# cityflow-project/CityFlow

Hardware: AMD Instinct MI355X
Metric: vehicle_steps_per_sec (higher is better)
Workload: dtype f64; 1 GPU; grid_30x30 (reference generator, --tlPlan, interval 1.0) + 3000 seeded interior flows (1 veh / 6 s each until t=240 s); single engine; running_vehicles_start=96748, running_vehicles_end=71131, lanes=11160, lane_count_hash_end=cf8592fdc74305bd, backend=hip-gfx950, layout=ring, parallelism=1 gpu

## Files before the change

### cityflow_amd/csrc/hip/cfx_device.h

```cpp
#pragma once

#include <hip/hip_runtime.h>
#include <stdint.h>

#include "cityflow_amd.h"

#define CFX_INT_MAX 2147483647

struct DevNet {
    int R, L, K, I, E;
    const double *drvLength, *drvMaxSpeed, *xDist, *phaseTime;
    const int32_t *laneRoad, *laneIndex, *laneLLStart, *laneLL, *llStartLane, *llEndLane, *llInter, *llRoadLink, *llType,
        *llXStart, *xPeer, *xLL, *interVirtual, *interNRL, *interPhaseStart, *interAvailStart;
    const uint8_t *phaseAvail;
    const int32_t *xPeerBit;
    const int32_t *llLocal;
    const int32_t *interMaskStart;
    const double2 *drvLM;
    const double2 *xDD;
    const int4 *xPack;
    const int4 *llPack;
    const int4 *laneLL4;
    const int4 *laneEnd4;
    const uint8_t *laneGhost;
// ... 107 lines not shown
        for (int k = 0; k < 8; ++k) curSpeedSum += v[k];
    }
    {
        double v[8];
#pragma unroll
        for (int k = 0; k < 8; ++k) v[k] = i + k < n ? speedAt(i + k) : 0.0;
#pragma unroll
        for (int k = 0; k < 8; ++k)
            if (i + k < n) curSpeedSum += v[k];
    }
    speedSum += curSpeedSum;
    int tail = head + len;
    if (tail >= kLaneHistoryMax) tail -= kLaneHistoryMax;
    h.num[(size_t) tail * h.L + lane] = n;
    h.avg[(size_t) tail * h.L + lane] = n ? curSpeedSum / n : 0;
    h.head[lane] = head;
    h.len[lane] = len + 1;
    h.hNum[lane] = hn;
    h.hAvg[lane] = hn ? speedSum / hn : 0;
}

struct TailRec {
    double dis, speed;
    int32_t slot, templ, prevDrv, tag;
};
static_assert(sizeof(TailRec) == 32, "tail record layout");

struct LLAux {
    double uDis, uSpeed, fDis, fSpeed, llLen, startLen;
    int32_t uTempl, fTempl;
};
static_assert(sizeof(LLAux) == 56, "laneLink aux record layout");

struct LeaverPrefetch {
    bool valid;
    double nextLen;
    int vid, route, routePos;
    bool prevValid;
    int prevDrv;
    int templP1;
    int blockerVidP2;
};

constexpr int kFlagCustom = 1, kFlagLastRoad = 2, kFlagStateGap = 4;
#ifndef CFX_CROSS2_WAVES
#define CFX_CROSS2_WAVES 7
#endif
struct StepCtx {
    static constexpr int kCross2Waves = CFX_CROSS2_WAVES;
    DevNet n;
    DevTables t;
    SlotArrays s;
    const int32_t *segStart;
    const int32_t *cnt;
    const int32_t *admitStep;
    int admissionsVisible;
    const int32_t *curPhase;
    const int32_t *oldToNew;
    const int32_t *vPriority;
    const double *vCustomSpeed;
    const double *vGapState;
    int4 *llDyn;
    unsigned long long *interMask;
    int2 *llGate;
    int32_t *laneTail;
    int2 *admitRec;
// ... 251 lines not shown
```

### cityflow_amd/csrc/hip/cfx_hip.hip

```cpp
#include <hip/hip_runtime.h>
#include <hip/hip_ext.h>

#include <algorithm>
#include <atomic>
#include <chrono>
#include <cmath>
#include <cstdio>
#include <cstring>
#include <map>
#include <string>
#include <thread>
#include <type_traits>
#include <vector>


#include "cfx_kernels.h"
#include "cfx_lc_kernels.h"
#include "cfx_ring_kernels.h"
#include "cfx_dense_kernels.h"

#ifndef CFX_CROSS2_BLOCKS_PER_CU
#define CFX_CROSS2_BLOCKS_PER_CU 7
#endif

// ... 174 lines not shown
        const int road = hLaneRoad[lane], base = hRouteStart[route], len = hRouteStart[route + 1] - base;
        int p = 0;
        while (p < len && hRouteRoads[base + p] != road) ++p;
        int next = -1;
        if (p < len) {
            const int ll = hNextLL[hNextStart[base + p] + hLaneIndex[lane]];
            next = ll < 0 ? -1 : L + ll;
        }
        if (next >= 0) return next;
        return (len > 0 && hRouteRoads[base + len - 1] == road) ? -2 : -1;
    }
    std::vector<int2> hRingGeo;
    size_t ringSlots = 0;
    double ringMinLen = 0.0;
    int ringScale = 1;
    int ringG = 14, ringCalm = 0, ringHold = 0;
    int2 *dRingGeo = nullptr;
    int32_t *rHead = nullptr, *rCnt = nullptr, *slotOf = nullptr;
    int4 *rScratch = nullptr;
    SlotArrays rs{};
    double2 *rKin[2] = {nullptr, nullptr};
    int4 *rMeta = nullptr;
    int rcur = 0;
    int2 *rBlk[2] = {nullptr, nullptr};
    TailRec *rTail[2] = {nullptr, nullptr}, *rTailNow = nullptr;
    MoverRec *rMovers = nullptr;
    long long *rFinKey = nullptr;
    int32_t *rFinVid = nullptr;
    double *rFinTerm = nullptr;
    int rFinCap = 0, rJobCap = 0;
    int32_t *rJobs = nullptr;
    RingJob *rJobRecs = nullptr;
    LLAux *rLLAux = nullptr;
    int4 *rLLGate = nullptr;
    int32_t *rGatePhase = nullptr;
    int4 *rList = nullptr;
    size_t rListCap = 0;
    int32_t *rListCount = nullptr;
    unsigned long long *rIdxGranules = nullptr;
    RingDense rd{};
    size_t rdCap = 0;
    int32_t *rOff = nullptr;

    bool timesDyadic = true;
    static bool dyadic(double x) { return x * 1024.0 == std::nearbyint(x * 1024.0) && std::fabs(x) < 4398046511104.0; }
    bool exactTimes() const {
        if (!timesDyadic) return false;
        const double cum = mirrorValid ? hMirror->sc.cumulativeTravelTime : cumLoaded;
        return dyadic(cum) && cum < 1099511627776.0;
    }
    double cumLoaded = 0.0;

    int64_t step = 0;
    int64_t finishedKnown = 0;
    int64_t finishedOffset = 0;

    bool profiling = false;
    std::vector<hipEvent_t> evPool;
    std::vector<int> evKernel;
    size_t evUsed = 0;
    double profMs[kNumProfKernels] = {};
    int64_t profLaunches[kNumProfKernels] = {};
    const char *slotSymbol[kNumProfKernels] = {};
    cfx_host_stats hostStats{};
    int stallCause = 0;

// ... 263 lines not shown
        RingCtx c{};
        c.tailR = rTail[(step + 1) & 1];
        c.tailW = rTail[step & 1];
        c.tailNow = rTailNow;
        c.betweenSteps = stepping ? 0 : 1;
        c.n = net;
        c.t.templ = dTempl.p;
        c.t.nTempl = (int) hTempl.size();
        c.t.routeStart = dRouteStart.p;
        c.t.routeRoads = dRouteRoads.p;
        c.t.nextStart = dNextStart.p;
        c.t.nextLL = dNextLL.p;
        c.s = rs;
        c.kin = rKin[rcur];
        c.kinN = rKin[rcur ^ 1];
        c.meta = rMeta;
        c.blkR = rBlk[(step + 1) & 1];
        c.blkW = rBlk[step & 1];
        c.slotOf = slotOf;
        c.vState = vt.state;
        c.ringGeo = dRingGeo;
        c.head = rHead;
        c.cnt = rCnt;
        c.admitStep = admitStep;
        c.curPhase = curPhase;
        c.vPriority = vt.priority;
        c.vCustomSpeed = vt.customSpeed;
        c.vGapState = vt.gapState;
        c.llDyn = llDyn;
        c.interMask = interMask;
        c.llGate = rLLGate;
        c.gatePhase = rGatePhase;
        c.llAux = rLLAux;
        c.laneTail = laneTail;
        c.admitRec = admitRec;
        c.step = (int32_t) step;
        c.interval = cfg.interval;
        return c;
    }
    template <typename T> int freeRaw(T **p) {
        if (*p) {
            forget(*p);
            HIP_TRY(hipFree(*p));
            *p = nullptr;
        }
        return CFX_OK;
    }
    int ringFree() {
        int rc = 0;
        rc |= freeRaw(&rs.vid) | freeRaw(&rs.drv) | freeRaw(&rs.prevDrv) | freeRaw(&rs.routePos) | freeRaw(&rs.route) |
              freeRaw(&rBlk[0]) | freeRaw(&rBlk[1]) | freeRaw(&rKin[0]) | freeRaw(&rKin[1]) | freeRaw(&rMeta) | freeRaw(&rMovers) |
              freeRaw(&dRingGeo) | freeRaw(&rJobs) | freeRaw(&rJobRecs);
        return rc ? CFX_ERR_DEVICE : CFX_OK;
    }
    int ringAllocate(double minLen) {
        hRingGeo.resize((size_t) D);
        size_t run = 0;
        for (int d = 0; d < D; ++d) {
            double want = std::ceil(hDrvLength[d] / minLen) + 6.0;
            if (cfg.ring_capacity_percent > 0) want = std::max(2.0, want * cfg.ring_capacity_percent / 100.0);
            want *= ringScale;
            size_t cap = 8;
            while ((double) cap < want && cap < (1u << (kRingIdxBits - 1))) cap <<= 1;
            run = (run + cap - 1) & ~(cap - 1);
            hRingGeo[d] = make_int2((int) run, (int) cap - 1);
            run += cap;
            if (run > 0x7fff0000u) return fail("ring layout: more than 2^31 slots");
        }
        ringSlots = run;
        ringMinLen = minLen;
        int rc;
#define RALLOC(ptr) if ((rc = allocRaw(&ptr, ringSlots))) return rc;
        RALLOC(rs.vid) RALLOC(rs.drv) RALLOC(rs.prevDrv) RALLOC(rs.routePos) RALLOC(rs.route)
        RALLOC(rBlk[0]) RALLOC(rBlk[1]) RALLOC(rKin[0]) RALLOC(rKin[1]) RALLOC(rMeta) RALLOC(rMovers)
#undef RALLOC
        HIP_TRY(hipMemsetAsync(rBlk[0], 0xFF, ringSlots * sizeof(int2), stream));
        HIP_TRY(hipMemsetAsync(rBlk[1], 0xFF, ringSlots * sizeof(int2), stream));
        HIP_TRY(hipMemsetAsync(rMeta, 0, ringSlots * sizeof(int4), stream));
        if ((rc = upload(&dRingGeo, hRingGeo.data(), hRingGeo.size()))) return rc;
        rJobCap = (int) std::max<size_t>(4096, ringSlots / 8);
        if ((rc = allocRaw(&rJobs, (size_t) rJobCap * kJobShards))) return rc;
        if ((rc = allocRaw(&rJobRecs, (size_t) rJobCap * kJobShards))) return rc;
        if (!rHead) {
            if ((rc = allocRaw(&rHead, (size_t) D + 1))) return rc;
            if ((rc = allocRaw(&rCnt, (size_t) D + 1))) return rc;
            if ((rc = allocRaw(&rOff, (size_t) D + 2))) return rc;
            if ((rc = allocRaw(&rScratch, (size_t) D))) return rc;
            if ((rc = allocRaw(&rTail[0], (size_t) D))) return rc;
            if ((rc = allocRaw(&rTail[1], (size_t) D))) return rc;
            if ((rc = allocRaw(&rTailNow, (size_t) D))) return rc;
            if ((rc = allocRaw(&rLLAux, (size_t) K))) return rc;
            if ((rc = allocRaw(&rLLGate, (size_t) K))) return rc;
            if ((rc = allocRaw(&rGatePhase, (size_t) 2 * std::max(I, 1)))) return rc;
            HIP_TRY(hipMemsetAsync(rGatePhase, 0xFF, (size_t) 2 * std::max(I, 1) * sizeof(int32_t), stream));
            rFinCap = std::max(1 << 16, L * 8);
            if ((rc = allocRaw(&rFinKey, (size_t) rFinCap))) return rc;
            if ((rc = allocRaw(&rFinVid, (size_t) rFinCap))) return rc;
            if ((rc = allocRaw(&rFinTerm, (size_t) rFinCap))) return rc;
            HIP_TRY(hipMemsetAsync(rCnt, 0, ((size_t) D + 1) * sizeof(int32_t), stream));
        }
        return CFX_OK;
    }
    int ensureDense(size_t n) {
        if (n <= rdCap) return CFX_OK;
        const size_t nc = std::max<size_t>(n + n / 4, 1 << 14);
        int rc;
        HIP_TRY(hipStreamSynchronize(stream));
#define DGROW(ptr) if ((rc = freeRaw(&ptr)) || (rc = allocRaw(&ptr, nc))) return rc;
        DGROW(rd.vid) DGROW(rd.drv) DGROW(rd.prevDrv) DGROW(rd.blockerVid) DGROW(rd.enterLLT) DGROW(rd.routePos) DGROW(rd.leaderVid)
        DGROW(rd.flags) DGROW(rd.dis) DGROW(rd.speed) DGROW(rd.gap)
#undef DGROW
        rdCap = nc;
        return CFX_OK;
    }
    int ringGather(bool wantLeader, int32_t *totalOut) {
        hipLaunchKernelGGL(kr_offsets, dim3(1), dim3(kOffBlock), 0, stream, (const int32_t *) rCnt, rOff, D + 1);
        int32_t total = 0;
        HIP_TRY(hipMemcpyAsync(&total, rOff + D, sizeof(int32_t), hipMemcpyDeviceToHost, stream));
        HIP_TRY(hipStreamSynchronize(stream));
        int rc = ensureDense((size_t) total);
        if (rc) return rc;
        if (total) hipLaunchKernelGGL(kr_gather, dim3(gridFor(D)), dim3(kBlock), 0, stream, rctx(), (const int32_t *) rOff, rd, wantLeader ? 1 : 0);
        HIP_TRY(hipGetLastError());
        *totalOut = total;
        return CFX_OK;
    }
    int ringClearStepTags() {
        HIP_TRY(hipMemsetAsync(rTailNow, 0xFF, (size_t) D * sizeof(TailRec), stream));
        HIP_TRY(hipMemsetAsync(interMask, 0, (size_t) std::max(nMaskWords, 1) * sizeof(unsigned long long), stream));
        return CFX_OK;
    }
    bool ringMerge = true;
    bool commitPending = false;
    size_t activeEstimate() const {
        const unsigned long long pr = __atomic_load_n(&hMirror->progress, __ATOMIC_RELAXED);
        return (size_t) (pr & 0xFFFFFFFFu) + (size_t) nQueueLanes * 4;
    }
    RingCommit commitArgs(size_t activeEst, bool lightsDone, int *nStatOut) {
        const int nStat = (int) std::min<size_t>(std::max<size_t>(1, activeEst >> 16), 64);
        *nStatOut = nStat;
        return RingCommit{rScratch, rMovers, waitHead, curPhase, remain, (int) cfg.rl_traffic_light, (int) nMaskWords,
                          sc, rFinKey, rFinVid, rFinTerm, rFinCap, jobCount,
                          hMirror, finTicket, nStat, vt.state, slotOf, exactTimes() ? 1 : 0,
                          lightsDone ? 1 : 0, publishTo(), finCount};
    }
    bool haloImportPending = false;
    RingHaloIn pendingImport{};
    bool histPending = false;
    RingHist takeHist(int firstBlock) {
        RingHist rh{};
        rh.firstBlock = 0x7fffffff;
        if (hist.num && ring && histPending) {
            rh.h = hist;
            rh.firstBlock = firstBlock;
            histPending = false;
        }
        return rh;
    }
    int settle(bool withHistory = true) {
        if (haloImportPending) {
            haloImportPending = false;
// ... 2542 lines not shown
    e->devObserveIdle = 0;
    return CFX_OK;
}

int32_t cfx_get_intersection_features(cfx_engine *e, int32_t *phase, double *remain, int32_t *in, int32_t *inWaiting, int32_t *out,
                                      int32_t *inside, int32_t *pressure, int32_t maxRoadLinks, int32_t maxPhases) {
    if (!e || (!phase && !remain && !in && !inWaiting && !out && !inside && !pressure)) return CFX_ERR_INVALID;
    auto fail = [e](const std::string &m) { return e->fail(m); };
    HIP_TRY(hipSetDevice(e->device));
    int rc;
    if ((rc = interPrepare(e, maxRoadLinks, maxPhases, "cfx_get_intersection_features"))) return rc;
    const size_t nI = (size_t) e->I, nM = nI * e->interTab.M, nP = nI * e->interTab.P;
    if (!e->interOutI && (rc = e->allocRaw(&e->interOutI, nI + 4 * nM + nP))) return rc;
    if (!e->interOutD && (rc = e->allocRaw(&e->interOutD, nI))) return rc;
    int32_t *dPhase = e->interOutI, *dIn = dPhase + nI, *dWait = dIn + nM, *dOut = dWait + nM, *dInside = dOut + nM,
            *dPressure = dInside + nM;
    launchInterFeatures(e, phase ? dPhase : nullptr, remain ? e->interOutD : nullptr, in ? dIn : nullptr, inWaiting ? dWait : nullptr,
                        out ? dOut : nullptr, inside ? dInside : nullptr, pressure ? dPressure : nullptr);
    HIP_TRY(hipGetLastError());
    auto back = [&](void *dst, const void *src, size_t bytes) {
        return (dst && bytes) ? hipMemcpyAsync(dst, src, bytes, hipMemcpyDeviceToHost, e->stream) : hipSuccess;
    };
    HIP_TRY(back(phase, dPhase, nI * sizeof(int32_t)));
    HIP_TRY(back(remain, e->interOutD, nI * sizeof(double)));
    HIP_TRY(back(in, dIn, nM * sizeof(int32_t)));
    HIP_TRY(back(inWaiting, dWait, nM * sizeof(int32_t)));
    HIP_TRY(back(out, dOut, nM * sizeof(int32_t)));
    HIP_TRY(back(inside, dInside, nM * sizeof(int32_t)));
    HIP_TRY(back(pressure, dPressure, nP * sizeof(int32_t)));
    HIP_TRY(hipStreamSynchronize(e->stream));
    return CFX_OK;
}

int32_t cfx_profile_kernel_count(void) { return kNumProfKernels; }
const char *cfx_profile_kernel_name(int32_t k) { return (k >= 0 && k < kNumProfKernels) ? kProfNames[k] : ""; }

int32_t cfx_profile_enable(cfx_engine *e, int32_t on) {
    if (!e) return CFX_ERR_INVALID;
    (void) hipSetDevice(e->device);
    if (e->profiling && !on) e->profCollect();
    e->profiling = on != 0;
    return CFX_OK;
}

int32_t cfx_profile_read(cfx_engine *e, double *totalMs, int64_t *launches) {
    if (!e) return CFX_ERR_INVALID;
    (void) hipSetDevice(e->device);
    e->profCollect();
    for (int k = 0; k < kNumProfKernels; ++k) {
        if (totalMs) totalMs[k] = e->profMs[k];
        if (launches) launches[k] = e->profLaunches[k];
        e->profMs[k] = 0;
        e->profLaunches[k] = 0;
    }
    return CFX_OK;
}

}
```

### cityflow_amd/csrc/hip/cfx_ring_kernels.h

```cpp
#pragma once

#include <type_traits>

#include "cfx_kernels.h"


namespace cfxd {

struct RingCtx {
#ifndef CFX_RING_CROSS2_WAVES
#define CFX_RING_CROSS2_WAVES 5
#endif
    static constexpr int kCross2Waves = CFX_RING_CROSS2_WAVES;
    DevNet n;
    DevTables t;
    SlotArrays s;
    double2 *kin;
    double2 *kinN;
    int4 *meta;
    const int2 *blkR;
    int2 *blkW;
    int32_t *slotOf;
    const uint8_t *vState;
    const int2 *ringGeo;
    const TailRec *tailR;
    TailRec *tailW;
    TailRec *tailNow;
    int betweenSteps;
    int32_t *head;
    int32_t *cnt;
    const int32_t *admitStep;
    const int32_t *curPhase;
    const int32_t *vPriority;
    const double *vCustomSpeed;
    const double *vGapState;
    int4 *llDyn;
    struct LLAux *llAux;
    unsigned long long *interMask;
    int4 *llGate;
    int32_t *gatePhase;
    int32_t *laneTail;
    int2 *admitRec;
    int32_t step;
    double interval;
};

__device__ __forceinline__ int ringSlot(const int2 geo, int head, int i) { return geo.x + ((head + i) & geo.y); }

__device__ __forceinline__ int committedCount(const RingCtx &c, int d) { return c.cnt[d]; }
__device__ __forceinline__ int cntNow(const RingCtx &c, int d) {
    return c.cnt[d] + ((d < c.n.L && c.admitStep[d] == c.step) ? 1 : 0);
}
__device__ __forceinline__ int firstSlot(const RingCtx &c, int d) { return ringSlot(c.ringGeo[d], c.head[d], 0); }
__device__ __forceinline__ int lastSlot(const RingCtx &c, int d) {
    const int n = cntNow(c, d);
    return n > 0 ? ringSlot(c.ringGeo[d], c.head[d], n - 1) : -1;
}
__device__ __forceinline__ int lastSlotForLeader(const RingCtx &c, int d, bool viewerNew, int viewerLane) {
    int n = c.cnt[d];
    if (viewerNew && d < viewerLane && d < c.n.L && c.admitStep[d] == c.step) n += 1;
    return n > 0 ? ringSlot(c.ringGeo[d], c.head[d], n - 1) : -1;
}
__device__ __forceinline__ Tail tailCommitted(const RingCtx &c, int d) {
    const TailRec r = c.tailR[d];
    Tail t = tailOfRec(r);
    if (r.tag != c.step - 1) t.slot = -1;
    return t;
}
__device__ __forceinline__ Tail tailNowOf(const RingCtx &c, int d) {
    if (c.betweenSteps) return tailCommitted(c, d);
// ... 686 lines not shown
    if (dyn.w > 0) {
        const SegWalk walk = segWalk(c, c.n.L + k, dyn.z);
        for (int i = 0; i < dyn.w; i += 2) {
            const int w0 = walk.at(i), w1 = walk.at(i + 1 < dyn.w ? i + 1 : i);
            const double2 k0 = c.kin[w0], k1 = c.kin[w1];
            const int t0 = c.meta[w0].x, t1 = c.meta[w1].x;
            for (int q = 0; q < 2 && i + q < dyn.w; ++q) {
                const int w = q ? w1 : w0;
                const double2 kw = q ? k1 : k0;
                const double vehDistance = kw.x;
                const int wt = q ? t1 : t0;
                if (!(vehDistance > x) || (vehDistance - x - tv[wt].len <= 0.0)) {
                    nf.slot = w;
                    nf.templ = wt;
                    nf.speed = kw.y;
                    nf.dist = x - vehDistance;
                    notifiedExtras(c, nf);
                    return nf;
                }
            }
        }
    }
    if (dyn.y >= 0) {
        nf.slot = dyn.y;
        nf.templ = a.fTempl;
        nf.speed = a.fSpeed;
        nf.dist = (a.startLen - a.fDis) + x;
        notifiedExtras(c, nf);
    }
    return nf;
}

__device__ inline Notified notifiedEagerFrom(const RingCtx &c, const cfx_vehicle_template *tv, int k, double x, const int4 dyn,
                                        const LLAux &a) {
    Notified nf{-1, 0, 0.0, 0.0, false, 0, make_int2(-1, -1)};
    if (dyn.x < 0 && dyn.y < 0 && dyn.w == 0) return nf;
    const SegWalk walk = segWalk(c, c.n.L + k, dyn.z);
    const bool haveU = dyn.x >= 0, haveOn = dyn.w > 0;
    const int w0 = haveOn ? walk.at(0) : 0, w1 = haveOn ? walk.at(dyn.w > 1 ? 1 : 0) : 0;
    double2 k0 = make_double2(0.0, 0.0), k1 = k0;
    int4 m0 = make_int4(0, 0, 0, 0), m1 = m0;
    int2 b0 = make_int2(-1, -1);
    int v0 = 0;
    if (haveOn) {
        k0 = c.kin[w0];
        k1 = c.kin[w1];
        m0 = c.meta[w0];
        m1 = c.meta[w1];
        b0 = c.blkR[w0];
        v0 = c.s.vid[w0];
    }
    if (haveU) {
        const double vehDistance = a.uDis - tv[a.uTempl].len;
        const double crossDistance = a.llLen - x;
        if (crossDistance + vehDistance < 0.0) {
            nf.slot = dyn.x;
            nf.templ = a.uTempl;
            nf.speed = a.uSpeed;
            nf.dist = -(a.uDis + crossDistance);
            notifiedExtras(c, nf);
            return nf;
        }
    }
    if (haveOn) {
        for (int q = 0; q < 2 && q < dyn.w; ++q) {
            const double2 kw = q ? k1 : k0;
            const int4 mw = q ? m1 : m0;
            const double vehDistance = kw.x;
            if (!(vehDistance > x) || (vehDistance - x - tv[mw.x].len <= 0.0)) {
                nf.slot = q ? w1 : w0;
                nf.templ = mw.x;
                nf.speed = kw.y;
                nf.dist = x - vehDistance;
                if (q == 0) {
                    nf.enterLLT = mw.w;
                    nf.blk = b0;
                    nf.vid = v0;
// ... 7 lines not shown
        for (int i = 2; i < dyn.w; i += 2) {
            const int x0 = walk.at(i), x1 = walk.at(i + 1 < dyn.w ? i + 1 : i);
            const double2 q0 = c.kin[x0], q1 = c.kin[x1];
            const int t0 = c.meta[x0].x, t1 = c.meta[x1].x;
            for (int q = 0; q < 2 && i + q < dyn.w; ++q) {
                const int w = q ? x1 : x0;
                const double2 kw = q ? q1 : q0;
                const double vehDistance = kw.x;
                const int wt = q ? t1 : t0;
                if (!(vehDistance > x) || (vehDistance - x - tv[wt].len <= 0.0)) {
                    nf.slot = w;
                    nf.templ = wt;
                    nf.speed = kw.y;
                    nf.dist = x - vehDistance;
                    notifiedExtras(c, nf);
                    return nf;
                }
            }
        }
    }
    if (dyn.y >= 0) {
        nf.slot = dyn.y;
        nf.templ = a.fTempl;
        nf.speed = a.fSpeed;
        nf.dist = (a.startLen - a.fDis) + x;
        notifiedExtras(c, nf);
    }
    return nf;
}

__device__ inline Notified notifiedEager(const RingCtx &c, const cfx_vehicle_template *tv, int k, double x) {
    const int4 dyn = c.llDyn[k];
    const LLAux a = c.llAux[k];
    return notifiedEagerFrom(c, tv, k, x, dyn, a);
}

struct RingJob {
    int32_t slot, d, idx, nNow, xs, xe, t1, templ, nd0, pad0, pad1, pad2;
    double d0, speed, v, iv, dis, dlen;
};
static_assert(sizeof(RingJob) == 96, "cross job record layout");

struct RingPush {
    JobQueue q;
    RingJob *recs;
    int L;
    __device__ __forceinline__ void operator()(int s, const JobInfo &j) const {
        const int shard = blockIdx.x & (kJobShards - 1);
        const int idx = jobQueuePlace(q);
        if (idx >= q.capacity) {
            *q.overflow = 9;
            return;
        }
        const size_t at = (size_t) shard * q.capacity + idx;
        q.jobs[at] = s;
        if (!recs) return;
        RingJob r{};
        r.slot = s;
        r.d = j.d;
        r.idx = j.idx;
        r.nNow = j.nNow;
        r.xs = j.xs;
        r.xe = j.xe;
        r.t1 = (j.gateFlags >> 1) & 3;
        r.templ = j.templ;
        r.nd0 = j.nd0;
        r.d0 = j.d < L ? -(j.dlen - j.dis) : j.dis;
// ... 389 lines not shown
    if (t == 0) sPre[0] = 0;
    __syncthreads();
    const int T = sPre[B];
    if (t == 0 && T > (B - 1) * 3 / 4) atomicMax(&o.sc->actionMaxT, T);
    TRACE_STAMP(1);
    const RingPush push{q, jobRecs, c.n.L};
    for (int qb = 0; qb < T; qb += B - 1) {
        const int qv = qb + t - 1;
        const bool valid = qv >= 0 && qv < T;
        int i = 0, idx = 0, slot = 0;
        SlotIn in;
        in.vid = -1;
        if (valid) {
            int lo = 0, hi = g;
            while (hi - lo > 1) {
                const int mid = (lo + hi) >> 1;
                if (sPre[mid] <= qv) lo = mid;
                else hi = mid;
            }
            i = lo;
            idx = qv - sPre[i];
            slot = ringSlot(sGeo[i], sHead[i], idx);
            const double2 kv = c.kin[slot];
            const int4 mv = c.meta[slot];
            in.dis = kv.x;
            in.speed = kv.y;
            in.templIdx = mv.x;
            in.nd0 = mv.y;
            in.flags = mv.z;
            in.lastRoadFlags = mv.z;
            sDis[t] = in.dis;
            sSpeed[t] = in.speed;
            sTempl[t] = in.templIdx;
        }
        __syncthreads();
        TRACE_STAMP(2);
        if (valid && t > 0) {
            in.vid = 0;
            in.d = d0 + i;
            in.head = idx == 0;
            in.idx = idx;
            in.nNow = sPre[i + 1] - sPre[i];
            in.leaderSlot = 0;
            if (idx > 0) {
                in.disPrev = sDis[t - 1];
                in.speedPrev = sSpeed[t - 1];
                in.templPrev = sTempl[t - 1];
                in.leaderSlot = ringSlot(sGeo[i], sHead[i], idx - 1);
            }
            if (in.flags & (kFlagCustom | kFlagStateGap)) {
                in.vid = c.s.vid[slot];
                c.meta[slot].z = in.flags & ~(kFlagCustom | kFlagStateGap);
            }
            in.lm = sLM[i];
            in.hop = (in.nd0 >= c.n.L) ? sHop[i] : make_int4(-2, -2, -2, -2);
            in.laneAdmitted = sAdm[i] != 0;
            in.endLane = -1;
            actionOneRounds<GHOST>(c, o, tv, slot, in, push);
        }
        __syncthreads();
        TRACE_STAMP(3);
    }
    TRACE_STAMP(4);
#ifdef CFX_TRACE
    if (t == 0) g_trace[(size_t) w * 8 + 5] = T;
#endif
// ... 827 lines not shown
```

### cityflow_amd/csrc/host/engine_host.cpp

```cpp
#include "engine_host.h"

#include <dlfcn.h>

#include <algorithm>
#include <chrono>
#include <climits>
#include <iostream>
#include <stdexcept>

#include "json.h"

namespace cfa {

std::string defaultBackendPath() {
    Dl_info info;
    if (dladdr((void *) &defaultBackendPath, &info) && info.dli_fname) {
        std::string p(info.dli_fname);
        size_t slash = p.find_last_of('/');
        std::string dir = slash == std::string::npos ? "." : p.substr(0, slash);
        return dir + "/lib/libcfx_hip.so";
    }
    return "libcfx_hip.so";
}

// ... 35 lines not shown
    CFX_FN(cfx_get_custom_speeds)
    CFX_FN(cfx_lane_change_supply)
    CFX_FN(cfx_lane_change_poll)
    CFX_FN(cfx_halo_config)
    CFX_FN(cfx_halo_export)
    CFX_FN(cfx_halo_import)
    CFX_FN(cfx_halo_attach)
    CFX_FN(cfx_halo_mailbox_alloc)
    CFX_FN(cfx_halo_mailbox_open)
    CFX_FN(cfx_halo_mailbox_fine_grained)
    CFX_FN(cfx_device_identity)
    CFX_FN(cfx_device_memory)
    CFX_FN(cfx_halo_device_buffers)
    CFX_FN(cfx_halo_post)
    CFX_FN(cfx_halo_wait)
    CFX_FN(cfx_profile_kernel_count)
    CFX_FN(cfx_profile_kernel_name)
    CFX_FN(cfx_profile_enable)
    CFX_FN(cfx_profile_read)
    CFX_FN(cfx_profile_kernel_symbol)
    CFX_FN(cfx_get_host_stats)
    CFX_FN(cfx_device_spin)
    CFX_FN(cfx_get_lane_history)
    CFX_FN(cfx_set_lane_history)
#undef CFX_FN
#define CFX_FN_OPTIONAL(name) name = reinterpret_cast<decltype(name)>(dlsym(handle, #name));
    CFX_FN_OPTIONAL(cfx_stream_handle)
    CFX_FN_OPTIONAL(cfx_set_tl_phases_device)
    CFX_FN_OPTIONAL(cfx_device_error)
    CFX_FN_OPTIONAL(cfx_observe_lanes_device)
    CFX_FN_OPTIONAL(cfx_get_lane_features)
    CFX_FN_OPTIONAL(cfx_observe_intersections_device)
    CFX_FN_OPTIONAL(cfx_get_intersection_features)
#undef CFX_FN_OPTIONAL
    if (cfx_abi_version() != CFX_ABI_VERSION)
        throw std::runtime_error("cityflow_amd: ABI version mismatch in '" + libPath + "'");
}

Backend::~Backend() {
    if (handle) dlclose(handle);
}

EngineConfig readEngineConfig(const std::string &configFile) {
    EngineConfig c;
    try {
        Json cfg = Json::parseFile(configFile);
        if (!cfg.isObject()) throw JsonError("wrong format of config file");
        c.interval = cfg.numberAt("interval");
        c.rlTrafficLight = cfg.boolAt("rlTrafficLight");
        c.laneChange = cfg.boolAt("laneChange", false);
        c.seed = cfg.intAt("seed");
        c.dir = cfg.stringAt("dir");
        c.roadnetFile = cfg.stringAt("roadnetFile");
        c.flowFile = cfg.stringAt("flowFile");
        c.saveReplay = cfg.boolAt("saveReplay");
        if (c.saveReplay) {
            c.roadnetLogFile = cfg.stringAt("roadnetLogFile");
            c.replayLogFile = cfg.stringAt("replayLogFile");
        }
        if (const Json *x = cfg.find("cfx")) {
            if (!x->isObject()) throw JsonError("cfx: expected an object");
            auto choice = [x](const char *key, std::initializer_list<const char *> names) {
                const Json *v = x->find(key);
                if (!v) return 0;
                if (!v->isString()) throw JsonError(std::string("cfx.") + key + ": expected a string");
                int i = 0;
// ... 926 lines not shown

void EngineHost::setTrafficLightPhaseOf(int inter, int phaseIndex) {
    if (!rlTrafficLight_) {
        std::cerr << "please set rlTrafficLight to true to enable traffic light control" << std::endl;
        return;
    }
    const HostInter &in = net_->inters.at((size_t) inter);
    if (in.isVirtual || phaseIndex < 0 || phaseIndex >= (int) in.phases.size())
        throw std::out_of_range("phase index " + std::to_string(phaseIndex) + " out of range for intersection '" + in.id + "'");
    pendingPhaseInter_.push_back(inter);
    pendingPhaseValue_.push_back(phaseIndex);
}

void EngineHost::trafficLightState(std::vector<int32_t> &phase, std::vector<double> &remain) {
    flushPhases();
    phase.resize(net_->inters.size());
    remain.resize(net_->inters.size());
    check(be_.cfx_get_tl_state(dev_, phase.data(), remain.data()), "cfx_get_tl_state");
    raiseDeviceError();
}

void EngineHost::laneHistory(std::vector<int32_t> &len, std::vector<int32_t> &vehicleNum, std::vector<double> &averageSpeed,
                             std::vector<int32_t> &historyVehicleNum, std::vector<double> &historyAverageSpeed) {
    const size_t nL = net_->lanes.size();
    len.assign(nL, 0);
    vehicleNum.assign(nL * CFX_LANE_HISTORY_MAX, 0);
    averageSpeed.assign(nL * CFX_LANE_HISTORY_MAX, 0.0);
    historyVehicleNum.assign(nL, 0);
    historyAverageSpeed.assign(nL, 0.0);
    cfx_lane_history h{(int32_t) nL, len.data(), vehicleNum.data(), averageSpeed.data(), historyVehicleNum.data(), historyAverageSpeed.data()};
    check(be_.cfx_get_lane_history(dev_, &h), "cfx_get_lane_history");
}

void EngineHost::setVehicleSpeed(const std::string &id, double speed) {
    dropAhead();
    int vid = vidOf(id);
    if (vid < 0) {
        const int future = spawner_.pendingPushedVid(id);
        if (future == -2) return;
        if (future >= 0) {
            check(be_.cfx_set_vehicle_speed(dev_, future, speed), "cfx_set_vehicle_speed");
            waitingCustom_[future] = speed;
            return;
        }
    }
    uint8_t st = 2;
    if (vid >= 0) check(be_.cfx_get_vehicle_status(dev_, vid, 1, &st), "cfx_get_vehicle_status");
    if (vid < 0 || st == 2) throw std::runtime_error("Vehicle '" + id + "' not found");
    check(be_.cfx_set_vehicle_speed(dev_, vid, speed), "cfx_set_vehicle_speed");
    if (st == 0) waitingCustom_[vid] = speed;
}

bool EngineHost::setRoute(const std::string &vehicleId, const std::vector<std::string> &anchorIds) {
    dropAhead();
    int vid = vidOf(vehicleId);
    if (vid < 0) return false;
    int32_t state = 2, drivable = -1, routePos = -1, route = -1;
    check(be_.cfx_get_vehicle(dev_, vid, &state, &drivable, &routePos, &route), "cfx_get_vehicle");
    if (state == 2) return false;
    std::vector<int> anchors;
    for (const auto &id : anchorIds) {
        auto it = net_->roadIndex.find(id);
        if (it == net_->roadIndex.end()) return false;
        anchors.push_back(it->second);
    }
    const int L = (int) net_->lanes.size();
// ... 59 lines not shown
```

### cityflow_amd/csrc/host/engine_host.h

```cpp
#pragma once

#include <map>
#include <memory>
#include <string>
#include <vector>

#include "archive.h"
#include "cityflow_amd.h"
#include "flow.h"
#include "replay.h"
#include "roadnet.h"

namespace cfa {

struct Backend {
    void *handle = nullptr;
    std::string path;
#define CFX_FN(name) decltype(&::name) name = nullptr;
    CFX_FN(cfx_abi_version)
    CFX_FN(cfx_create)
    CFX_FN(cfx_destroy)
    CFX_FN(cfx_last_error)
    CFX_FN(cfx_backend_name)
    CFX_FN(cfx_add_templates)
// ... 21 lines not shown
    CFX_FN(cfx_lane_change_poll)
    CFX_FN(cfx_halo_config)
    CFX_FN(cfx_halo_export)
    CFX_FN(cfx_halo_import)
    CFX_FN(cfx_halo_attach)
    CFX_FN(cfx_halo_mailbox_alloc)
    CFX_FN(cfx_halo_mailbox_open)
    CFX_FN(cfx_halo_mailbox_fine_grained)
    CFX_FN(cfx_device_identity)
    CFX_FN(cfx_device_memory)
    CFX_FN(cfx_halo_device_buffers)
    CFX_FN(cfx_halo_post)
    CFX_FN(cfx_halo_wait)
    CFX_FN(cfx_profile_kernel_count)
    CFX_FN(cfx_profile_kernel_name)
    CFX_FN(cfx_profile_enable)
    CFX_FN(cfx_profile_read)
    CFX_FN(cfx_profile_kernel_symbol)
    CFX_FN(cfx_get_host_stats)
    CFX_FN(cfx_device_spin)
    CFX_FN(cfx_get_lane_history)
    CFX_FN(cfx_set_lane_history)
#undef CFX_FN
    cfx_stream_handle_fn cfx_stream_handle = nullptr;
    cfx_observe_lanes_device_fn cfx_observe_lanes_device = nullptr;
    cfx_set_tl_phases_device_fn cfx_set_tl_phases_device = nullptr;
    cfx_device_error_fn cfx_device_error = nullptr;
    bool hasDeviceBuffers() const {
        return cfx_stream_handle && cfx_observe_lanes_device && cfx_set_tl_phases_device && cfx_device_error;
    }
    cfx_get_lane_features_fn cfx_get_lane_features = nullptr;
    cfx_observe_intersections_device_fn cfx_observe_intersections_device = nullptr;
    cfx_get_intersection_features_fn cfx_get_intersection_features = nullptr;
    void open(const std::string &libPath);
    ~Backend();
};

enum SnapshotField : unsigned {
    kSnapDrivable = 1, kSnapPrev = 2, kSnapLeader = 4, kSnapBlocker = 8, kSnapEnterLL = 16, kSnapRoutePos = 32,
    kSnapDis = 64, kSnapSpeed = 128, kSnapGap = 256, kSnapAll = 511,
    kSnapLaneChange = 512
};

struct VehicleSnapshot {
    std::vector<int32_t> vid, drivable, prevDrivable, leader, blocker, enterLLTime, routePos;
    std::vector<double> dis, speed, gap;
    std::vector<int32_t> lcPartner, lcLastDir, lcTarget, lcDirection;
    std::vector<uint8_t> lcFlags;
    std::vector<double> lcOffset, lcLastChangeTime, lcWaitingTime;
    int count = 0;
    bool isShadow(int i) const { return !lcFlags.empty() && (lcFlags[i] & CFX_LC_SHADOW); }
};

struct InterLayout {
    int I = 0, M = 0, P = 0, Kin = 0, Kout = 0;
    std::vector<int32_t> nRoadLinks, nPhases;
    std::vector<uint8_t> phaseAvail;
    std::vector<int32_t> roadLinkType;
    std::vector<int32_t> inLanes, outLanes;
    std::vector<int32_t> llRow;
};
InterLayout intersectionLayoutOf(const HostRoadNet &net);
struct InterFeatures {
    int32_t *phase = nullptr;
    double *remain = nullptr;
    int32_t *in = nullptr, *inWaiting = nullptr, *out = nullptr, *inside = nullptr, *pressure = nullptr;
// ... 41 lines not shown
    void setReplayLogFile(const std::string &logFile);
    void setSaveReplay(bool open);

    std::vector<int32_t> laneVehicleCountArray();
    std::vector<int32_t> laneWaitingVehicleCountArray();
    std::vector<std::string> laneIds() const;
    const std::vector<int32_t> &laneIdOrder();
    std::vector<std::string> intersectionIds() const;
    void setTrafficLightPhaseIndexed(int inter, int phase);
    void setTrafficLightPhases(const std::vector<int32_t> &phases);
    void setTrafficLightPhases(const int32_t *phases, size_t n);
    void trafficLightState(std::vector<int32_t> &phase, std::vector<double> &remain);
    bool deviceBuffers() const { return be_.hasDeviceBuffers(); }
    std::pair<uintptr_t, int> streamHandle();
    void setTrafficLightPhasesDevice(uintptr_t phases, size_t n, uintptr_t producerStream);
    bool rlTrafficLight() const { return rlTrafficLight_; }
    std::vector<int32_t> phaseCounts() const;
    std::vector<double> laneLengths() const;
    void laneFeatures(double *speedSum, int32_t *bins, const double *edges, int nBins, bool perLaneEdges);
    void observeLanesDevice(uintptr_t counts, uintptr_t waiting, uintptr_t speedSum, uintptr_t bins, uintptr_t edges, int nBins,
                            bool perLaneEdges, uintptr_t consumerStream);
    const InterLayout &intersectionLayout();
    void intersectionFeatures(const InterFeatures &out);
    void observeIntersectionsDevice(uintptr_t phase, uintptr_t remain, uintptr_t in, uintptr_t inWaiting, uintptr_t out,
                                    uintptr_t inside, uintptr_t pressure, int maxRoadLinks, int maxPhases, uintptr_t consumerStream);
    void laneHistory(std::vector<int32_t> &len, std::vector<int32_t> &vehicleNum, std::vector<double> &averageSpeed,
                     std::vector<int32_t> &historyVehicleNum, std::vector<double> &historyAverageSpeed);
    void snapshotVehicles(VehicleSnapshot &out, unsigned fields = kSnapAll);
    uint64_t vehicleEpoch() const { return vehicleEpoch_; }
    void waitingVehicles(std::vector<int32_t> &vid, std::vector<int32_t> &lane);
    cfx_scalars scalars();
    void sync();
    void profileEnable(bool on);
    void deviceSpin(long long microseconds) { check(be_.cfx_device_spin(dev_, microseconds), "cfx_device_spin"); }
    std::pair<long long, long long> deviceMemory() {
        int64_t f = 0, t = 0;
        check(be_.cfx_device_memory(dev_, &f, &t), "cfx_device_memory");
        return {(long long) f, (long long) t};
    }
    std::map<std::string, std::pair<double, int64_t>> profileRead();
    std::map<std::string, std::string> profileSymbols();
    cfx_host_stats hostStats(bool reset);
    struct SlowestStep {
        double total = 0, part[6] = {};
        int64_t step = -1;
    };
    SlowestStep slowestStep(bool reset) {
        SlowestStep s = slowest_;
        if (reset) slowest_ = SlowestStep{};
        return s;
    }

    std::shared_ptr<void> bindingCache;

    const HostRoadNet &net() const { return *net_; }
    const Spawner &spawner() {
        dropAhead();
        return spawner_;
    }
    std::string backendName() const { return be_.cfx_backend_name ? be_.cfx_backend_name() : "?"; }
    std::pair<int64_t, int> ringInfo() {
        int64_t slots = 0;
        int32_t scale = 1;
        be_.cfx_get_ring_info(dev_, &slots, &scale);
        return {slots, scale};
    }
// ... 80 lines not shown
```

### cityflow_amd/csrc/host/pymodule.cpp

```cpp
#include <pybind11/functional.h>
#include <pybind11/numpy.h>
#include <pybind11/pybind11.h>
#include <pybind11/stl.h>

#include <chrono>
#include <iostream>

#include "archive.h"
#include "engine_host.h"
#include "tile_engine.h"
#include "vector_engine.h"
#include "json.h"

namespace py = pybind11;
using namespace py::literals;
using cfa::EngineHost;

namespace {

template <typename T> py::array_t<T> toArray(const std::vector<T> &v) {
    py::array_t<T> a((py::ssize_t) v.size());
    if (!v.empty()) std::memcpy(a.mutable_data(), v.data(), v.size() * sizeof(T));
    return a;
}
template <typename T> py::array_t<T> toArray(const T *p, size_t n) {
    py::array_t<T> a((py::ssize_t) n);
    if (n) std::memcpy(a.mutable_data(), p, n * sizeof(T));
    return a;
}

py::dict flatNetToDict(const cfa::HostRoadNet &net) {
    const cfx_net &f = net.flat();
// ... 507 lines not shown
                     d["lc_flags"] = toArray(s.lcFlags);
                     d["lc_offset"] = toArray(s.lcOffset);
                     d["lc_last_dir"] = toArray(s.lcLastDir);
                     d["lc_target"] = toArray(s.lcTarget);
                     d["lc_direction"] = toArray(s.lcDirection);
                     d["lc_last_change_time"] = toArray(s.lcLastChangeTime);
                 }
                 return d;
             })
        .def("_waiting",
             [](EngineHost &e) {
                 std::vector<int32_t> v, l;
                 e.waitingVehicles(v, l);
                 return py::make_tuple(toArray(v), toArray(l));
             })
        .def("_keeps_lane_history", &EngineHost::keepsLaneHistory)
        .def("_compact_vehicles", &EngineHost::compactVehicles,
             "forget the finished vehicles now (automatic once \"cfx\": {\"compactVehicles\": N} vehicles have been created; default 3.5 M)")
        .def("_vehicle_table", [](EngineHost &e) { return py::make_tuple(e.vehicleTableSize(), e.vehicleCompactions()); },
             "(vehicle numbers the host holds, compactions so far)")
        .def("_lane_history",
             [](EngineHost &e) {
                 std::vector<int32_t> len, num, hn;
                 std::vector<double> avg, ha;
                 e.laneHistory(len, num, avg, hn, ha);
                 py::dict d;
                 d["len"] = toArray(len);
                 d["vehicle_num"] = toArray(num);
                 d["average_speed"] = toArray(avg);
                 d["history_vehicle_num"] = toArray(hn);
                 d["history_average_speed"] = toArray(ha);
                 return d;
             })
        .def("_tl_state",
             [](EngineHost &e) {
                 std::vector<int32_t> p;
                 std::vector<double> r;
                 e.trafficLightState(p, r);
                 return py::make_tuple(toArray(p), toArray(r));
             })
        .def("_scalars",
             [](EngineHost &e) {
                 cfx_scalars s = e.scalars();
                 py::dict d;
                 d["step"] = s.step;
                 d["active_vehicle_count"] = s.active_vehicle_count;
                 d["finished_vehicle_count"] = s.finished_vehicle_count;
                 d["spawned_vehicle_count"] = s.spawned_vehicle_count;
                 d["cumulative_travel_time"] = s.cumulative_travel_time;
                 d["live_enter_time_sum"] = s.live_enter_time_sum;
                 d["vehicle_steps"] = s.vehicle_steps;
                 d["tie_events"] = s.tie_events;
                 py::list td;
                 for (int i = 0; i < 8; ++i)
                     if (s.tie_drivables[i] >= 0) td.append(s.tie_drivables[i]);
                 d["tie_drivables"] = td;
                 d["diag_cross_jobs"] = s.diag_cross_jobs;
                 d["dropped_future_speeds"] = s.dropped_future_speeds;
                 return d;
             })
        .def("_layout", &EngineHost::layoutName)
        .def("_ring_info", &EngineHost::ringInfo, "(total ring slots, capacity scale) of the ring layout")
        .def("_profile_enable", &EngineHost::profileEnable, "on"_a)
        .def("_device_spin", &EngineHost::deviceSpin, "microseconds"_a)
        .def("_device_memory", &EngineHost::deviceMemory, "(free, total) bytes of the engine's device")
        .def("_profile_read", &EngineHost::profileRead)
// ... 324 lines not shown
```

### include/cityflow_amd.h

```cpp
#ifndef CITYFLOW_AMD_H
#define CITYFLOW_AMD_H

#include <stdint.h>

#ifdef __cplusplus
extern "C" {
#endif

#define CFX_ABI_VERSION 9

typedef enum cfx_status {
    CFX_OK = 0,
    CFX_ERR_INVALID = -1,
    CFX_ERR_DEVICE = -2,
    CFX_ERR_CAPACITY = -3,
    CFX_ERR_STATE = -4
} cfx_status;

typedef struct cfx_engine cfx_engine;

typedef struct cfx_net {
    int32_t n_roads, n_lanes, n_lanelinks, n_inters;
    int32_t n_xentries;
    int32_t n_phases;
// ... 241 lines not shown
typedef struct cfx_host_stats {
    int64_t step_calls;
    double step_call_us_sum;
    double worst_step_call_us;
    int64_t worst_step_call_at;
    int32_t worst_step_call_cause;
    int32_t calls_over_1ms;
    int64_t ring_regrows_total;
    int64_t table_grows_total;
    double worst_status_query_us, worst_status_query_settle_us, worst_status_query_copy_us, worst_status_query_wait_us;
    int64_t status_queries;
} cfx_host_stats;
int32_t cfx_get_host_stats(cfx_engine *e, cfx_host_stats *out, int32_t reset);
int32_t cfx_device_spin(cfx_engine *e, int64_t microseconds);

typedef int32_t (*cfx_stream_handle_fn)(cfx_engine *e, void **stream, int32_t *device);
typedef int32_t (*cfx_observe_device_fn)(cfx_engine *e, int32_t *counts, int32_t *waiting, void *consumer_stream);
typedef int32_t (*cfx_set_tl_phases_device_fn)(cfx_engine *e, const int32_t *phases, int32_t n, void *producer_stream);
typedef int32_t (*cfx_device_error_fn)(cfx_engine *e, int32_t *inter, int32_t *phase);

typedef int32_t (*cfx_observe_lanes_device_fn)(cfx_engine *e, int32_t *counts, int32_t *waiting, double *speed_sum, int32_t *bins,
                                               const double *edges, int32_t n_bins, int32_t per_lane_edges, void *consumer_stream);
typedef int32_t (*cfx_get_lane_features_fn)(cfx_engine *e, double *speed_sum, int32_t *bins, const double *edges, int32_t n_bins,
                                            int32_t per_lane_edges);
#define CFX_MAX_LANE_BINS 32

typedef int32_t (*cfx_observe_intersections_device_fn)(cfx_engine *e, int32_t *phase, double *remain, int32_t *in, int32_t *in_waiting,
                                                       int32_t *out, int32_t *inside, int32_t *phase_pressure, int32_t max_roadlinks,
                                                       int32_t max_phases, void *consumer_stream);
typedef int32_t (*cfx_get_intersection_features_fn)(cfx_engine *e, int32_t *phase, double *remain, int32_t *in, int32_t *in_waiting,
                                                    int32_t *out, int32_t *inside, int32_t *phase_pressure, int32_t max_roadlinks,
                                                    int32_t max_phases);

#ifdef __cplusplus
}
#endif
#endif
```

Measured before the change: 1.980 billion vehicle-steps/s.

## Cache laneLink head vehicle state in packed 64-byte records for eager notification

Adds a per-laneLink 64-byte LLHead record that the lane pass fills with the first two vehicles' kinematics, template, enter time, vid and blocker. notifiedEagerFrom then reads this single contiguous record, tagged with the current step, instead of gathering from the kin/meta/blk/vid slot arrays. The goal is to replace scattered dependent loads with one coalesced line. It costs extra writes in the lane kernel plus a per-step memset of K records. A debug export path is also added.

```diff
diff --git a/cityflow_amd/csrc/hip/cfx_device.h b/cityflow_amd/csrc/hip/cfx_device.h
--- a/cityflow_amd/csrc/hip/cfx_device.h
+++ b/cityflow_amd/csrc/hip/cfx_device.h
@@ -163,6 +163,12 @@
 };
 static_assert(sizeof(LLAux) == 56, "laneLink aux record layout");
 
+struct alignas(64) LLHead {
+    double dis0, speed0, dis1, speed1;
+    int32_t templ0, enterLLT0, vid0, blk0x, blk0y, tag, templ1, pad;
+};
+static_assert(sizeof(LLHead) == 64, "laneLink head record layout");
+
 struct LeaverPrefetch {
     bool valid;
     double nextLen;
diff --git a/cityflow_amd/csrc/hip/cfx_hip.hip b/cityflow_amd/csrc/hip/cfx_hip.hip
--- a/cityflow_amd/csrc/hip/cfx_hip.hip
+++ b/cityflow_amd/csrc/hip/cfx_hip.hip
@@ -230,6 +230,7 @@
     int32_t *rJobs = nullptr;
     RingJob *rJobRecs = nullptr;
     LLAux *rLLAux = nullptr;
+    LLHead *rLLHead = nullptr;
     int4 *rLLGate = nullptr;
     int32_t *rGatePhase = nullptr;
     int4 *rList = nullptr;
@@ -559,6 +560,7 @@
         c.llGate = rLLGate;
         c.gatePhase = rGatePhase;
         c.llAux = rLLAux;
+        c.llHead = rLLHead;
         c.laneTail = laneTail;
         c.admitRec = admitRec;
         c.step = (int32_t) step;
@@ -617,6 +619,8 @@
             if ((rc = allocRaw(&rTail[1], (size_t) D))) return rc;
             if ((rc = allocRaw(&rTailNow, (size_t) D))) return rc;
             if ((rc = allocRaw(&rLLAux, (size_t) K))) return rc;
+            if ((rc = allocRaw(&rLLHead, (size_t) K))) return rc;
+            HIP_TRY(hipMemsetAsync(rLLHead, 0xFF, (size_t) K * sizeof(LLHead), stream));
             if ((rc = allocRaw(&rLLGate, (size_t) K))) return rc;
             if ((rc = allocRaw(&rGatePhase, (size_t) 2 * std::max(I, 1)))) return rc;
             HIP_TRY(hipMemsetAsync(rGatePhase, 0xFF, (size_t) 2 * std::max(I, 1) * sizeof(int32_t), stream));
@@ -654,6 +658,7 @@
     }
     int ringClearStepTags() {
         HIP_TRY(hipMemsetAsync(rTailNow, 0xFF, (size_t) D * sizeof(TailRec), stream));
+        HIP_TRY(hipMemsetAsync(rLLHead, 0xFF, (size_t) K * sizeof(LLHead), stream));
         HIP_TRY(hipMemsetAsync(interMask, 0, (size_t) std::max(nMaskWords, 1) * sizeof(unsigned long long), stream));
         return CFX_OK;
     }
@@ -3262,6 +3267,22 @@
     return CFX_OK;
 }
 
+int32_t cfx_debug_cross_head_records(cfx_engine *e, void *records, int32_t nLaneLinks);
+static_assert(std::is_same<decltype(&cfx_debug_cross_head_records), cfx_debug_cross_head_records_fn>::value,
+              "cfx_debug_cross_head_records");
+int32_t cfx_debug_cross_head_records(cfx_engine *e, void *records, int32_t nLaneLinks) {
+    if (!e || !records || !e->ring || nLaneLinks != e->K) return CFX_ERR_INVALID;
+    if (!e->rLLHead) {
+        memset(records, 0xFF, (size_t) e->K * sizeof(LLHead));
+        return CFX_OK;
+    }
+    auto fail = [e](const std::string &m) { return e->fail(m); };
+    HIP_TRY(hipSetDevice(e->device));
+    HIP_TRY(hipMemcpyAsync(records, e->rLLHead, (size_t) e->K * sizeof(LLHead), hipMemcpyDeviceToHost, e->stream));
+    HIP_TRY(hipStreamSynchronize(e->stream));
+    return CFX_OK;
+}
+
 int32_t cfx_profile_kernel_count(void) { return kNumProfKernels; }
 const char *cfx_profile_kernel_name(int32_t k) { return (k >= 0 && k < kNumProfKernels) ? kProfNames[k] : ""; }
 
diff --git a/cityflow_amd/csrc/hip/cfx_ring_kernels.h b/cityflow_amd/csrc/hip/cfx_ring_kernels.h
--- a/cityflow_amd/csrc/hip/cfx_ring_kernels.h
+++ b/cityflow_amd/csrc/hip/cfx_ring_kernels.h
@@ -36,6 +36,7 @@
     const double *vGapState;
     int4 *llDyn;
     struct LLAux *llAux;
+    struct LLHead *llHead;
     unsigned long long *interMask;
     int4 *llGate;
     int32_t *gatePhase;
@@ -788,7 +789,7 @@
 }
 
 __device__ inline Notified notifiedEagerFrom(const RingCtx &c, const cfx_vehicle_template *tv, int k, double x, const int4 dyn,
-                                        const LLAux &a) {
+                                        const LLAux &a, const LLHead &hr) {
     Notified nf{-1, 0, 0.0, 0.0, false, 0, make_int2(-1, -1)};
     if (dyn.x < 0 && dyn.y < 0 && dyn.w == 0) return nf;
     const SegWalk walk = segWalk(c, c.n.L + k, dyn.z);
@@ -798,7 +799,15 @@
     int4 m0 = make_int4(0, 0, 0, 0), m1 = m0;
     int2 b0 = make_int2(-1, -1);
     int v0 = 0;
-    if (haveOn) {
+    if (haveOn && hr.tag == c.step) {
+        k0 = make_double2(hr.dis0, hr.speed0);
+        m0.x = hr.templ0;
+        m0.w = hr.enterLLT0;
+        b0 = make_int2(hr.blk0x, hr.blk0y);
+        v0 = hr.vid0;
+        k1 = dyn.w > 1 ? make_double2(hr.dis1, hr.speed1) : k0;
+        m1.x = dyn.w > 1 ? hr.templ1 : hr.templ0;
+    } else if (haveOn) {
         k0 = c.kin[w0];
         k1 = c.kin[w1];
         m0 = c.meta[w0];
@@ -872,7 +881,8 @@
 __device__ inline Notified notifiedEager(const RingCtx &c, const cfx_vehicle_template *tv, int k, double x) {
     const int4 dyn = c.llDyn[k];
     const LLAux a = c.llAux[k];
-    return notifiedEagerFrom(c, tv, k, x, dyn, a);
+    const LLHead hr = c.llHead[k];
+    return notifiedEagerFrom(c, tv, k, x, dyn, a, hr);
 }
 
 struct RingJob {
@@ -1328,6 +1338,25 @@
             sDis[t] = in.dis;
             sSpeed[t] = in.speed;
             sTempl[t] = in.templIdx;
+            if (!laneBlock && idx < 2 && t > 0) {
+                LLHead *const hr = c.llHead + (d0 + i - c.n.L);
+                if (idx == 0) {
+                    const int2 bl = c.blkR[slot];
+                    const int vid = c.s.vid[slot];
+                    hr->dis0 = kv.x;
+                    hr->speed0 = kv.y;
+                    hr->templ0 = mv.x;
+                    hr->enterLLT0 = mv.w;
+                    hr->vid0 = vid;
+                    hr->blk0x = bl.x;
+                    hr->blk0y = bl.y;
+                    hr->tag = c.step;
+                } else {
+                    hr->dis1 = kv.x;
+                    hr->speed1 = kv.y;
+                    hr->templ1 = mv.x;
+                }
+            }
         }
         __syncthreads();
         TRACE_STAMP(2);
diff --git a/cityflow_amd/csrc/host/engine_host.cpp b/cityflow_amd/csrc/host/engine_host.cpp
--- a/cityflow_amd/csrc/host/engine_host.cpp
+++ b/cityflow_amd/csrc/host/engine_host.cpp
@@ -91,6 +91,7 @@
     CFX_FN_OPTIONAL(cfx_get_lane_features)
     CFX_FN_OPTIONAL(cfx_observe_intersections_device)
     CFX_FN_OPTIONAL(cfx_get_intersection_features)
+    CFX_FN_OPTIONAL(cfx_debug_cross_head_records)
 #undef CFX_FN_OPTIONAL
     if (cfx_abi_version() != CFX_ABI_VERSION)
         throw std::runtime_error("cityflow_amd: ABI version mismatch in '" + libPath + "'");
@@ -1083,6 +1084,13 @@
     check(be_.cfx_get_lane_history(dev_, &h), "cfx_get_lane_history");
 }
 
+std::vector<unsigned char> EngineHost::crossHeadRecords() {
+    if (!be_.cfx_debug_cross_head_records) throw std::runtime_error("this backend keeps no laneLink head records");
+    std::vector<unsigned char> raw(net_->laneLinks.size() * 64);
+    check(be_.cfx_debug_cross_head_records(dev_, raw.data(), (int32_t) net_->laneLinks.size()), "cfx_debug_cross_head_records");
+    return raw;
+}
+
 void EngineHost::setVehicleSpeed(const std::string &id, double speed) {
     dropAhead();
     int vid = vidOf(id);
diff --git a/cityflow_amd/csrc/host/engine_host.h b/cityflow_amd/csrc/host/engine_host.h
--- a/cityflow_amd/csrc/host/engine_host.h
+++ b/cityflow_amd/csrc/host/engine_host.h
@@ -77,6 +77,7 @@
     cfx_get_lane_features_fn cfx_get_lane_features = nullptr;
     cfx_observe_intersections_device_fn cfx_observe_intersections_device = nullptr;
     cfx_get_intersection_features_fn cfx_get_intersection_features = nullptr;
+    cfx_debug_cross_head_records_fn cfx_debug_cross_head_records = nullptr;
     void open(const std::string &libPath);
     ~Backend();
 };
@@ -184,6 +185,7 @@
     cfx_scalars scalars();
     void sync();
     void profileEnable(bool on);
+    std::vector<unsigned char> crossHeadRecords();
     void deviceSpin(long long microseconds) { check(be_.cfx_device_spin(dev_, microseconds), "cfx_device_spin"); }
     std::pair<long long, long long> deviceMemory() {
         int64_t f = 0, t = 0;
diff --git a/cityflow_amd/csrc/host/pymodule.cpp b/cityflow_amd/csrc/host/pymodule.cpp
--- a/cityflow_amd/csrc/host/pymodule.cpp
+++ b/cityflow_amd/csrc/host/pymodule.cpp
@@ -1,3 +1,4 @@
+#include <cstring>
 #include <pybind11/functional.h>
 #include <pybind11/numpy.h>
 #include <pybind11/pybind11.h>
@@ -571,6 +572,25 @@
                  d["history_average_speed"] = toArray(ha);
                  return d;
              })
+        .def("_cross_head_records",
+             [](EngineHost &e) {
+                 const std::vector<unsigned char> raw = e.crossHeadRecords();
+                 const size_t K = raw.size() / 64;
+                 static const char *const dn[4] = {"dis0", "speed0", "dis1", "speed1"};
+                 static const char *const in[7] = {"templ0", "enter_ll_time0", "vid0", "blocker_vid0", "blocker_step0", "tag", "templ1"};
+                 py::dict d;
+                 for (int f = 0; f < 4; ++f) {
+                     std::vector<double> col(K);
+                     for (size_t k = 0; k < K; ++k) std::memcpy(&col[k], &raw[k * 64 + 8 * f], 8);
+                     d[dn[f]] = toArray(col);
+                 }
+                 for (int f = 0; f < 7; ++f) {
+                     std::vector<int32_t> col(K);
+                     for (size_t k = 0; k < K; ++k) std::memcpy(&col[k], &raw[k * 64 + 32 + 4 * f], 4);
+                     d[in[f]] = toArray(col);
+                 }
+                 return d;
+             })
         .def("_tl_state",
              [](EngineHost &e) {
                  std::vector<int32_t> p;
diff --git a/include/cityflow_amd.h b/include/cityflow_amd.h
--- a/include/cityflow_amd.h
+++ b/include/cityflow_amd.h
@@ -297,6 +297,8 @@
                                                     int32_t *out, int32_t *inside, int32_t *phase_pressure, int32_t max_roadlinks,
                                                     int32_t max_phases);
 
+typedef int32_t (*cfx_debug_cross_head_records_fn)(cfx_engine *e, void *records, int32_t n_lanelinks);
+
 #ifdef __cplusplus
 }
 #endif
```

Result: slower. 1.935 billion vehicle-steps/s (-2.3%).
